# vincenthz/eccoxide

Measured on AMD Instinct MI355X. Metric: variable-base scalarmuls/sec (batch) per GPU + achieved HBM GB/s vs roofline, higher is better.
Workload: dtype u32

## Files before the change

### __graft_entry__.py

```python
import os
import subprocess
import sys

ROOT = os.path.dirname(os.path.abspath(__file__))
if ROOT not in sys.path:
    sys.path.insert(0, ROOT)


def build() -> None:
    jobs = str(min(6, os.cpu_count() or 1))
    subprocess.check_call(["make", "-C", os.path.join(ROOT, "eccoxide_amd", "csrc"), "-j", jobs, "ARCH=gfx950"])
    subprocess.check_call(["make", "-C", os.path.join(ROOT, "oracle")])
    subprocess.check_call(["make", "-C", os.path.join(ROOT, "tests", "cpp")])
    subprocess.check_call(["make", "-C", os.path.join(ROOT, "tests", "hip")])
    subprocess.check_call(["make", "-C", os.path.join(ROOT, "tests", "hip_p256k1")])
    subprocess.check_call(["make", "-C", os.path.join(ROOT, "tests", "hip_ed25519")])
    subprocess.check_call(["make", "-C", os.path.join(ROOT, "tests", "hip_merged")])
    subprocess.check_call(["make", "-C", os.path.join(ROOT, "tests", "hip_lo32")])
    subprocess.check_call(["make", "-C", os.path.join(ROOT, "tests", "hip_ecdsa")])
    subprocess.check_call(["make", "-C", os.path.join(ROOT, "tests", "hip_ed25519_sign")])
    subprocess.check_call(["make", "-C", os.path.join(ROOT, "tests", "hip_ecdsa_sign")])
    subprocess.check_call(["make", "-C", os.path.join(ROOT, "tests", "hip_h2c")])
    subprocess.check_call(["make", "-C", os.path.join(ROOT, "tests", "hip_g2")])
    subprocess.check_call(["make", "-C", os.path.join(ROOT, "tests", "hip_h2c_g2")])
    import eccoxide_amd
    from eccoxide_amd import _lib

    lib = _lib.load()
    assert lib.eccx_field_bytes(eccoxide_amd.P256R1) == 32


def smoke() -> None:
    import eccoxide_amd as E
    from eccoxide_amd import workload as W
    from tests import oracle_lib

    ora = oracle_lib.load()
    with E.Engine(0) as eng:
        for curve, n in (("p256r1", 300), ("ed25519", 300)):
            ks = W.random_scalars(curve, n, seed=1).tobytes()
            want_b = ora.base(curve, ks, threads=4)
            got_b = eng.scalarmul_base(curve, ks)
            assert got_b[0] == want_b[0] and got_b[1] == want_b[1], f"{curve}: fixed-base mismatch vs oracle"
            pts = want_b[0]
            ks2 = W.random_scalars(curve, n, seed=2).tobytes()
            want_v = ora.var(curve, ks2, pts, threads=4)
            got_d = eng.scalarmul_var(curve, ks2, pts)
            assert got_d[0] == want_v[0] and got_d[1] == want_v[1], f"{curve}: variable-base mismatch vs oracle"
            got_v = eng.scalarmul_var(curve, ks2, pts, want_proj=True)
            assert got_v[0] == want_v[0] and got_v[1] == want_v[1], f"{curve}: mirror variable-base mismatch vs oracle"
# ... 78 lines not shown
```

### eccoxide_amd/csrc/kernels_coz.hpp

```cpp
#pragma once
#include <type_traits>
#include "inv_gcd.hpp"
#include "kernels_ct.hpp"

namespace eccx {

struct NoGlv {
  static constexpr int K_BITS = 0;
};
struct PrimeOrderBases : NoGlv {};

template <class G>
ECCX_DEV void glv_split(uint32_t (&k1)[5], uint32_t (&k2)[5], const uint8_t* __restrict__ kb) {
  uint32_t k[8];
#pragma unroll
  for (int i = 0; i < 8; ++i) {
    const uint8_t* b = kb + 28 - 4 * i;
    k[i] = ((uint32_t)b[0] << 24) | ((uint32_t)b[1] << 16) | ((uint32_t)b[2] << 8) | (uint32_t)b[3];
  }
  uint32_t prod[13];
#pragma unroll
  for (int i = 0; i < 13; ++i) prod[i] = 0;
#pragma unroll
  for (int i = 0; i < 8; ++i) {
// ... 200 lines not shown
  constexpr uint32_t T = TAGGED ? CT_F32_TAG : 0u;
  uint32_t w[W];
#pragma unroll
  for (int i = 0; i < W; ++i) w[i] = (i < N ? x.v[i] : (i < 2 * N ? y.v[i - N] : 0u)) | T;
  uint4* dst = reinterpret_cast<uint4*>(row);
#pragma unroll
  for (int i = 0; i < W / 4; ++i) dst[i] = make_uint4(w[4 * i], w[4 * i + 1], w[4 * i + 2], w[4 * i + 3]);
}

template <class CU>
ECCX_DEV void ujac_madd_signed(UJac<CU>& r, bool& h_zero, bool& r_zero, const UJac<CU>& p,
                          const U<CU, 1, 3>& x2, const U<CU, 1, 3>& y2, bool neg) {
  auto z1z1 = u_sqr(p.z);
  auto u2 = u_mul(x2, z1z1);
  auto t = u_mul(p.z, z1z1);
  U<CU, 2, 4> sy;
  u_select(sy, neg, u_neg(y2), u_as<2, 4>(y2));
  auto s2 = u_mul(u_reduce(sy), t);
  auto h = u_reduce(u_sub(u2, p.x));
  auto rr = u_reduce(u_sub(s2, p.y));
  h_zero = u_is_zero_mod_p(h);
  r_zero = u_is_zero_mod_p(rr);
  auto hh = u_sqr(h);
  auto hhh = u_mul(h, hh);
  auto v = u_mul(p.x, hh);
  auto r2 = u_sqr(rr);
  auto x3 = u_reduce(u_sub(u_sub(u_sub(r2, hhh), v), v));
  r.x = x3;
  if constexpr (CU::KIND == UK_MONT) {
    r.y = u_fit<1, 3>(u_mul_add(rr, u_sub(v, x3), u_neg(p.y), hhh));
  } else if constexpr (UB<CU>::SPARSE) {
    r.y = u_mul_sub(rr, u_sub(v, x3), p.y, hhh);
  } else if constexpr (UBS<CU>::DENSE) {
    r.y = u_mul_sub(rr, u_reduce(u_sub(v, x3)), p.y, hhh);
  } else {
    auto y3a = u_mul(rr, u_sub(v, x3));
    auto y1h = u_mul(p.y, hhh);
    r.y = u_reduce(u_sub(y3a, y1h));
  }
  r.z = u_fit<UJac<CU>::ZK, UJac<CU>::ZV>(u_mul(p.z, h));
}

template <class CU>
ECCX_DEV void uzaddu(U<CU, 1, 3>& x1, U<CU, 1, 3>& y1, U<CU, 1, 3>& x2, U<CU, 1, 3>& y2, U<CU, 1, 3>& d_out, bool& d_zero) {
  const auto d = u_reduce(u_sub(x1, x2));
  d_zero = u_is_zero_mod_p(d);
  const auto c = u_sqr(d);
  const U<CU, 1, 3> w1 = u_fit<1, 3>(u_mul(x1, c));
  const auto w2 = u_mul(x2, c);
  const auto e = u_reduce(u_sub(y1, y2));
  const auto dd = u_sqr(e);
  const U<CU, 1, 3> a1 = u_fit<1, 3>(u_mul(y1, u_sub(w1, w2)));
  const auto x3 = u_reduce(u_sub(u_sub(dd, w1), w2));
  const auto y3m = u_mul(e, u_sub(w1, x3));
  x2 = x3;
  y2 = u_reduce(u_sub(y3m, a1));
  x1 = w1;
  y1 = a1;
  d_out = d;
}

template <class CU>
ECCX_DEV void ujac_madd_ct(UJac<CU>& r, bool& h_zero, bool& r_zero, const UJac<CU>& p, const U<CU, 1, 3>& x2,
                           const U<CU, 1, 3>& y2) {
  auto z1z1 = u_sqr(p.z);
  auto u2 = u_mul(x2, z1z1);
  auto t = u_mul(p.z, z1z1);
// ... 515 lines not shown
```

### eccoxide_amd/csrc/kernels_unsat.hpp

```cpp
#pragma once
#include "kernels_fast.hpp"
#include "ufe.hpp"

namespace eccx {
#ifndef ECCX_ENTRY_ALIGN
#define ECCX_ENTRY_ALIGN 32
#endif

template <class CU>
struct UJac {
  static constexpr int ZK = UB<CU>::KLAZY, ZV = ZK == 2 ? 4 : 3;
  U<CU, 1, 3> x, y;
  U<CU, ZK, ZV> z;
};

template <class CU>
struct UEntry {
  U<CU, 1, 3> x, y, z, zz, zzz;
};

template <class CU>
constexpr int urow3_words() { return ((3 * CU::N + 3) / 4) * 4; }
template <class CU>
ECCX_DEV void u3_store(uint32_t* __restrict__ row, const U<CU, 1, 3>& x, const U<CU, 1, 3>& y, const U<CU, 1, 3>& z) {
// ... 71 lines not shown
    r.x = x3;
    r.y = u_reduce(u_sub(u_sub(y3m, gg4), gg4));
    r.z = u_fit<UJac<CU>::ZK, UJac<CU>::ZV>(u_add(yz, yz));
  } else {
    auto delta = u_sqr(p.z);
    auto gamma = u_sqr(p.y);
    auto g2 = u_add(gamma, gamma);
    auto g4 = u_add(g2, g2);
    auto b4 = u_mul(p.x, g4);
    auto t1 = u_sub(p.x, delta);
    auto t2 = u_add(p.x, delta);
    auto t3 = u_mul(t1, t2);
    auto alpha = u_reduce(u_add(u_add(t3, t3), t3));
    auto x3a = u_sqr(alpha);
    auto x3 = u_reduce(u_sub(u_sub(x3a, b4), b4));
    auto yz = u_mul(p.y, p.z);
    auto t = u_sub(b4, x3);
    r.x = x3;
    if constexpr (UB<CU>::SPARSE) {
      r.y = u_mul_sub_2sqr(alpha, t, g2);
    } else {
      auto g8s = u_sqr(g2);
      auto y3m = u_mul(alpha, t);
      r.y = u_reduce(u_sub(u_sub(y3m, g8s), g8s));
    }
    r.z = u_fit<UJac<CU>::ZK, UJac<CU>::ZV>(u_add(yz, yz));
  }
}

template <class CU>
ECCX_DEV void ujac_dbl_merged(UJac<CU>& r, const UJac<CU>& p) {
  static_assert(UBS<CU>::DENSE && !CU::Sat::A0, "written for a = -3 on p = -1 mod 2^B without the sparse form");
  auto delta = u_sqr(p.z);
  auto gamma = u_sqr(p.y);
  auto g2 = u_reduce(u_add(gamma, gamma));
  auto g4 = u_add(g2, g2);
  auto b4 = u_mul(p.x, g4);
  auto t1 = u_sub(p.x, delta);
  auto t2 = u_add(p.x, delta);
  auto t3 = u_mul(t1, t2);
  auto alpha = u_reduce(u_add(u_add(t3, t3), t3));
  auto x3 = u_reduce(u_sub(u_sub(u_sqr(alpha), b4), b4));
  auto yz = u_mul(p.y, p.z);
  r.x = x3;
  r.y = u_mul_sub_2sqr(alpha, u_reduce(u_sub(b4, x3)), g2);
  r.z = u_fit<UJac<CU>::ZK, UJac<CU>::ZV>(u_add(yz, yz));
}

template <class CU>
ECCX_DEV void ujac_add_raw(UJac<CU>& r, bool& h_zero, bool& r_zero, U<CU, 1, 3>& ey, const UJac<CU>& p,
                           const UEntry<CU>& e, bool neg) {
  auto z1z1 = u_sqr(p.z);
  auto u1 = u_mul(p.x, e.zz);
  auto u2 = u_mul(e.x, z1z1);
  auto s1 = u_mul(p.y, e.zzz);
  auto t = u_mul(p.z, z1z1);
  U<CU, 2, 4> sy;
  u_select(sy, neg, u_neg(e.y), u_as<2, 4>(e.y));
  ey = u_reduce(sy);
  auto s2 = u_mul(ey, t);
  auto h = u_reduce(u_sub(u2, u1));
  auto rr = u_reduce(u_sub(s2, s1));
  h_zero = u_is_zero_mod_p(h);
  r_zero = u_is_zero_mod_p(rr);
  auto hh = u_sqr(h);
  auto hhh = u_mul(h, hh);
  auto v = u_mul(u1, hh);
  auto r2 = u_sqr(rr);
  auto x3 = u_reduce(u_sub(u_sub(u_sub(r2, hhh), v), v));
  auto tt = u_sub(v, x3);
  auto z3a = u_mul(p.z, e.z);
  r.x = x3;
  if constexpr (CU::KIND == UK_MONT) {
    r.y = u_fit<1, 3>(u_mul_add(rr, tt, u_neg(s1), hhh));
  } else if constexpr (UB<CU>::SPARSE) {
    r.y = u_mul_sub(rr, tt, s1, hhh);
  } else {
    auto y3a = u_mul(rr, tt);
// ... 1317 lines not shown
```

### eccoxide_amd/csrc/ufe.hpp

```cpp
#pragma once
#include "fe.hpp"

#include <type_traits>

#ifndef ECCX_SOLINAS_REDUCE
#define ECCX_SOLINAS_REDUCE 1
#endif

namespace eccx {

#include "umad_chunks.inc"

__device__ __forceinline__ void smad1_k(uint64_t& acc, uint32_t a, int32_t k) {
  asm("v_mad_i64_i32 %0, vcc, %1, %2, %0" : "+v"(acc) : "v"(a), "s"(k) : "vcc");
}

__device__ __forceinline__ void smad1_v(uint64_t& acc, int32_t a, int32_t b) {
  asm("v_mad_i64_i32 %0, vcc, %1, %2, %0" : "+v"(acc) : "v"(a), "v"(b) : "vcc");
}

template <int S>
__device__ __forceinline__ void ucarry_hi(uint64_t& acc) {
  uint64_t r;
  asm("v_mad_u64_u32 %0, vcc, %1, %2, 0" : "=&v"(r) : "v"((uint32_t)(acc >> 32)), "n"(1 << S) : "vcc");
// ... 123 lines not shown
  switch (q.n) {                                                                                                     \
    case 1: umad1_##SUF<F>(acc, h, ECCX_Q(0)); break;                                                              \
    case 2: umad2_##SUF<F>(acc, h, ECCX_Q(0), ECCX_Q(1)); break;                                                   \
    case 3: umad3_##SUF<F>(acc, h, ECCX_Q(0), ECCX_Q(1), ECCX_Q(2)); break;                                        \
    case 4: umad4_##SUF<F>(acc, h, ECCX_Q(0), ECCX_Q(1), ECCX_Q(2), ECCX_Q(3)); break;                             \
    case 5: umad5_##SUF<F>(acc, h, ECCX_Q(0), ECCX_Q(1), ECCX_Q(2), ECCX_Q(3), ECCX_Q(4)); break;                  \
    case 6: umad6_##SUF<F>(acc, h, ECCX_Q(0), ECCX_Q(1), ECCX_Q(2), ECCX_Q(3), ECCX_Q(4), ECCX_Q(5)); break;       \
    case 7: umad7_##SUF<F>(acc, h, ECCX_Q(0), ECCX_Q(1), ECCX_Q(2), ECCX_Q(3), ECCX_Q(4), ECCX_Q(5), ECCX_Q(6));   \
      break;                                                                                                       \
    case 8:                                                                                                        \
      umad8_##SUF<F>(acc, h, ECCX_Q(0), ECCX_Q(1), ECCX_Q(2), ECCX_Q(3), ECCX_Q(4), ECCX_Q(5), ECCX_Q(6), ECCX_Q(7)); \
      break;                                                                                                       \
    case 9:                                                                                                        \
      umad9_##SUF<F>(acc, h, ECCX_Q(0), ECCX_Q(1), ECCX_Q(2), ECCX_Q(3), ECCX_Q(4), ECCX_Q(5), ECCX_Q(6), ECCX_Q(7), \
                     ECCX_Q(8));                                                                                   \
      break;                                                                                                       \
    default:                                                                                                       \
      if (hc == 2) scarry_hi<S>(acc);                                                                              \
      else ucarry_hi<S>(acc);                                                                                      \
      break;                                                                                                       \
  }
    if constexpr (KC) {
      if (hc == 2) { ECCX_CHUNKS(ks) } else { ECCX_CHUNKS(kc) }
    } else {
      if (hc == 2) { ECCX_CHUNKS(vs) } else { ECCX_CHUNKS(vc) }
    }
#undef ECCX_CHUNKS
#undef ECCX_Q
    q.n = 0;
    hc = 0;
  }
};


template <class C, bool SQR, bool BCONST, bool LO32 = UB<C>::LO32>
ECCX_DEV void u_mul_core_mont(uint32_t (&r)[C::N], const uint32_t (&a)[C::N], const uint32_t (&b)[C::N]) {
  constexpr int N = C::N;
  constexpr bool PP1 = C::KIND == UK_MONT_PP1;
  auto PR = [](int j) constexpr { return PP1 ? C::PP1[j] : C::P[j]; };
  uint32_t m[N], t[N], a2[N];
  if constexpr (SQR) {
#pragma unroll
    for (int i = 0; i < N; ++i) a2[i] = a[i] << 1;
  }
  uint64_t acc = 0;
  std::conditional_t<UB<C>::LO32, UMacQC<BCONST, 32 - C::B>, UMacQ<BCONST>> qa;
  UMacQ<true> qm;
#pragma unroll
  for (int k = 0; k < 2 * N - 1; ++k) {
    const int lo = k < N ? 0 : k - N + 1, hi = k < N ? k : N - 1;
    if constexpr (SQR) {
#pragma unroll
      for (int i = lo; 2 * i < k; ++i) qa.push(acc, a[i], a2[k - i]);
      if ((k & 1) == 0) qa.push(acc, a[k / 2], a[k / 2]);
    } else {
#pragma unroll
      for (int i = lo; i <= hi; ++i) qa.push(acc, a[i], b[k - i]);
    }
    qa.flush(acc);
    if constexpr (UB<C>::SPARSE) {
#pragma unroll
      for (int t = 0; t < C::SPARSE_N; ++t) {
        const int i = k - C::SPARSE_OFF[t];
        if (i >= lo && i <= (k < N ? k - 1 : N - 1)) {
          if (C::SPARSE_SIGN[t] > 0) qm.push(acc, m[i], 1u << C::SPARSE_SHIFT[t]);
        }
      }
      qm.flush(acc);
#pragma unroll
      for (int t = 0; t < C::SPARSE_N; ++t) {
        const int i = k - C::SPARSE_OFF[t];
        if (i >= lo && i <= (k < N ? k - 1 : N - 1)) {
          if (C::SPARSE_SIGN[t] < 0) smad1_k(acc, m[i], -(int32_t)(1u << C::SPARSE_SHIFT[t]));
        }
      }
    } else {
#pragma unroll
      for (int i = lo; i <= (k < N ? k - 1 : N - 1); ++i) {
        if (PR(k - i) != 0) qm.push(acc, m[i], PR(k - i));
      }
      qm.flush(acc);
    }
    if constexpr (LO32) {
      if (k < N - 1) {
// ... 129 lines not shown
  for (int k = 0; k < 2 * N - 1; ++k) {
    const int lo = k < N ? 0 : k - N + 1, hi = k < N ? k : N - 1;
    if (k >= N) acc += (uint64_t)C::P[k - N];
#pragma unroll
    for (int i = lo; i <= hi; ++i) qa.push(acc, a[i], b[k - i]);
    qa.flush(acc);
    if constexpr (NEG_SQ) {
#pragma unroll
      for (int i = lo; 2 * i < k; ++i) smad1_v(acc, nc[i], (int32_t)(c[k - i] << 1));
      if ((k & 1) == 0) smad1_v(acc, nc[k / 2], (int32_t)c[k / 2]);
    } else {
#pragma unroll
      for (int i = lo; i <= hi; ++i) smad1_v(acc, nc[i], (int32_t)d[k - i]);
    }
#pragma unroll
    for (int i = lo; i <= (k < N ? k - 1 : N - 1); ++i) {
      if (C::P[k - i] != 0) qm.push(acc, m[i], C::P[k - i]);
    }
    qm.flush(acc);
    if (k < N) {
      m[k] = ((uint32_t)acc * C::N0B) & C::MASK;
      umad1_k(acc, m[k], C::P[0]);
    } else {
      t[k - N] = (uint32_t)acc & C::MASK;
    }
    acc = (uint64_t)((int64_t)acc >> C::B);
  }
  acc += (uint64_t)C::P[N - 1];
  t[N - 1] = (uint32_t)acc;
#pragma unroll
  for (int i = 0; i < N; ++i) r[i] = t[i];
}

template <class C, bool NEG_SQ>
ECCX_DEV void u_mul_sub_core_pp1(uint32_t (&r)[C::N], const uint32_t (&a)[C::N], const uint32_t (&b)[C::N],
                                 const uint32_t (&c)[C::N], const uint32_t (&d)[C::N]) {
  constexpr int N = C::N;
  static_assert(C::KIND == UK_MONT_PP1 && C::SPARSE_N == 0, "p = -1 mod 2^B with p + 1 as plain digits");
  uint32_t m[N], t[N];
  int32_t nc[N];
#pragma unroll
  for (int i = 0; i < N; ++i) nc[i] = NEG_SQ ? -(int32_t)(c[i] << 1) : -(int32_t)c[i];
  uint64_t acc = 0;
  UMacQC<false, 32 - C::B> qa;
  UMacQ<true> qm;
#pragma unroll
  for (int k = 0; k < 2 * N - 1; ++k) {
    const int lo = k < N ? 0 : k - N + 1, hi = k < N ? k : N - 1;
    if (k >= N && C::P[k - N] != 0) acc += (uint64_t)C::P[k - N];
#pragma unroll
    for (int i = lo; i <= hi; ++i) qa.push(acc, a[i], b[k - i]);
    qa.flush(acc);
    if constexpr (NEG_SQ) {
#pragma unroll
      for (int i = lo; 2 * i < k; ++i) smad1_v(acc, nc[i], (int32_t)(c[k - i] << 1));
      if ((k & 1) == 0) smad1_v(acc, nc[k / 2], (int32_t)c[k / 2]);
    } else {
#pragma unroll
      for (int i = lo; i <= hi; ++i) smad1_v(acc, nc[i], (int32_t)d[k - i]);
    }
#pragma unroll
    for (int i = lo; i <= (k < N ? k - 1 : N - 1); ++i) {
      if (C::PP1[k - i] != 0) qm.push(acc, m[i], C::PP1[k - i]);
    }
    qm.flush(acc);
    if (k < N - 1) {
      m[k] = (uint32_t)acc;
      qa.carry(acc, true);
      continue;
    }
    if (k < N) m[k] = (uint32_t)acc & C::MASK;
    else t[k - N] = (uint32_t)acc & C::MASK;
    acc = (uint64_t)((int64_t)acc >> C::B);
  }
  acc += (uint64_t)C::P[N - 1];
  t[N - 1] = (uint32_t)acc;
#pragma unroll
  for (int i = 0; i < N; ++i) r[i] = t[i];
}

template <class C, bool SQR, bool BCONST>
ECCX_DEV void u_mul_core_mers(uint32_t (&r)[C::N], const uint32_t (&a)[C::N], const uint32_t (&b)[C::N]) {
  constexpr int N = C::N;
  constexpr int S = C::B * N - C::PBITS;
  static_assert(S >= 1 && S <= 2, "wrap factor must keep shifted limbs below 2^32");
  uint32_t t[N], bw[N], a2[N];
#pragma unroll
  for (int i = 0; i < N; ++i) {
    if constexpr (SQR) {
      a2[i] = a[i] << 1;
      bw[i] = (S == 1) ? 0u : a[i] << (S + 1);
    } else {
      a2[i] = 0;
      bw[i] = b[i] << S;
    }
  }
  uint64_t acc = 0;
  UMacQ<BCONST && !SQR> qa;
  UMacQ<false> qw;
#pragma unroll
  for (int k = 0; k < N; ++k) {
// ... 197 lines not shown
  static constexpr bool DENSE = C::KIND == UK_MONT_PP1 && !UB<C>::SPARSE;
  static constexpr int KKS = (int)((~(uint64_t)0 >> 1) / ((uint64_t)C::N * UB<C>::COL)) - 1;
  static_assert(!DENSE || (uint64_t)C::N * KKS * UB<C>::COL <= (~(uint64_t)0 >> 1) - 0xffffffffull * UB<C>::pp1_sum() -
                                                                ((uint64_t)1 << C::B) - ((uint64_t)1 << (63 - C::B)),
                "32-bit Montgomery digits overflow the signed columns");
  static constexpr bool ks_ok(int k) { return ((uint64_t)(k + 1) << C::B) <= ((uint64_t)1 << 31); }
};

template <class C, int K1, int V1, int K2, int V2, int K3, int V3, int K4, int V4>
ECCX_DEV auto u_mul_sub(const U<C, K1, V1>& a, const U<C, K2, V2>& b, const U<C, K3, V3>& c, const U<C, K4, V4>& d) {
  static_assert(UBS<C>::OK || UBS<C>::DENSE, "implemented for the Montgomery fields with room for signed columns");
  static_assert(K1 * K2 <= UBS<C>::KKS && K3 * K4 <= UBS<C>::KKS, "a product overflows the signed columns");
  static_assert(UBS<C>::ks_ok(K3) && UBS<C>::ks_ok(K4), "negated / signed operands must stay below 2^31");
  static_assert((uint32_t)(V1 * V2) < C::RP && (uint32_t)(V3 * V4) < C::RP, "result outside (0, 3p)");
  U<C, 1, 3> r;
  if constexpr (UB<C>::SPARSE) u_mul_sub_core_sparse<C, false>(r.v, a.v, b.v, c.v, d.v);
  else if constexpr (UBS<C>::DENSE) u_mul_sub_core_pp1<C, false>(r.v, a.v, b.v, c.v, d.v);
  else u_mul_sub_core_mont<C, false>(r.v, a.v, b.v, c.v, d.v);
  return r;
}
template <class C, int K1, int V1, int K2, int V2, int K3, int V3>
ECCX_DEV auto u_mul_sub_2sqr(const U<C, K1, V1>& a, const U<C, K2, V2>& b, const U<C, K3, V3>& c) {
  static_assert(UBS<C>::OK || UBS<C>::DENSE, "implemented for the Montgomery fields with room for signed columns");
  static_assert(K1 * K2 <= UBS<C>::KKS && 2 * K3 * K3 <= UBS<C>::KKS, "a product overflows the signed columns");
  static_assert(UBS<C>::ks_ok(2 * K3), "doubled / negated operands must stay below 2^31");
  static_assert((uint32_t)(V1 * V2) < C::RP && (uint32_t)(2 * V3 * V3) < C::RP, "result outside (0, 3p)");
  U<C, 1, 3> r;
  if constexpr (UB<C>::SPARSE) u_mul_sub_core_sparse<C, true>(r.v, a.v, b.v, c.v, c.v);
  else if constexpr (UBS<C>::DENSE) u_mul_sub_core_pp1<C, true>(r.v, a.v, b.v, c.v, c.v);
  else u_mul_sub_core_mont<C, true>(r.v, a.v, b.v, c.v, c.v);
  return r;
}

template <class C, int K1, int V1>
ECCX_DEV auto u_sqr(const U<C, K1, V1>& a) {
  if constexpr (!UB<C>::ksq_ok(K1) || (UB<C>::vout(V1, V1) > 3)) {
    return u_sqr(u_reduce(a));
  } else {
    U<C, 1, UB<C>::vout(V1, V1)> r;
    u_mul_core<C, true, false>(r.v, a.v, a.v);
    return r;
  }
}

template <class C, int K1, int V1>
ECCX_DEV auto u_mul_k(const U<C, K1, V1>& a, const uint32_t (&k)[C::N]) {
  if constexpr (!UB<C>::kk_ok(K1, 1) || (UB<C>::vout(V1, 1) > 3)) {
    return u_mul_k(u_reduce(a), k);
  } else {
    U<C, 1, UB<C>::vout(V1, 1)> r;
    u_mul_core<C, false, true>(r.v, a.v, k);
    return r;
  }
}

template <class C>
ECCX_DEV U<C, 1, 2> u_mul_k_exit(const U<C, 1, 3>& a, const uint32_t (&k)[C::N]) {
  static_assert(UB<C>::MONT && UB<C>::vout(3, 1) <= 2, "Montgomery fields; a reduced operand times a constant below p");
  U<C, 1, 2> r;
  u_mul_core_mont<C, false, true, false>(r.v, a.v, k);
  return r;
}

template <class C, int K1, int V1>
ECCX_DEV U<C, 1, 2> u_mul_small(const U<C, K1, V1>& a, uint32_t k) {
  static_assert(C::KIND == UK_PM19, "written for 2^255 - 19");
// ... 217 lines not shown
```

### eccoxide_amd/csrc/umad_chunks.inc

```
__device__ __forceinline__ void umad1_v(uint64_t& acc, uint32_t a0, uint32_t b0) {
  asm("v_mad_u64_u32 %0, vcc, %1, %2, %0\n\t"
      : "+v"(acc)
      : "v"(a0), "v"(b0)
      : "vcc");
}
__device__ __forceinline__ void umad2_v(uint64_t& acc, uint32_t a0, uint32_t b0, uint32_t a1, uint32_t b1) {
  asm("v_mad_u64_u32 %0, vcc, %1, %2, %0\n\t"
      "v_mad_u64_u32 %0, vcc, %3, %4, %0\n\t"
      : "+v"(acc)
      : "v"(a0), "v"(b0), "v"(a1), "v"(b1)
      : "vcc");
}
__device__ __forceinline__ void umad3_v(uint64_t& acc, uint32_t a0, uint32_t b0, uint32_t a1, uint32_t b1, uint32_t a2, uint32_t b2) {
  asm("v_mad_u64_u32 %0, vcc, %1, %2, %0\n\t"
      "v_mad_u64_u32 %0, vcc, %3, %4, %0\n\t"
      "v_mad_u64_u32 %0, vcc, %5, %6, %0\n\t"
      : "+v"(acc)
      : "v"(a0), "v"(b0), "v"(a1), "v"(b1), "v"(a2), "v"(b2)
      : "vcc");
}
__device__ __forceinline__ void umad4_v(uint64_t& acc, uint32_t a0, uint32_t b0, uint32_t a1, uint32_t b1, uint32_t a2, uint32_t b2, uint32_t a3, uint32_t b3) {
  asm("v_mad_u64_u32 %0, vcc, %1, %2, %0\n\t"
      "v_mad_u64_u32 %0, vcc, %3, %4, %0\n\t"
      "v_mad_u64_u32 %0, vcc, %5, %6, %0\n\t"
// ... 554 lines not shown
      : "vcc");
}
template <int F>
__device__ __forceinline__ void umad8_ks(uint64_t& acc, uint32_t h, uint32_t a0, uint32_t b0, uint32_t a1, uint32_t b1, uint32_t a2, uint32_t b2, uint32_t a3, uint32_t b3, uint32_t a4, uint32_t b4, uint32_t a5, uint32_t b5, uint32_t a6, uint32_t b6, uint32_t a7, uint32_t b7) {
  asm("v_mad_i64_i32 %0, vcc, %1, %2, 0\n\t"
      "v_mad_u64_u32 %0, vcc, %3, %4, %0\n\t"
      "v_mad_u64_u32 %0, vcc, %5, %6, %0\n\t"
      "v_mad_u64_u32 %0, vcc, %7, %8, %0\n\t"
      "v_mad_u64_u32 %0, vcc, %9, %10, %0\n\t"
      "v_mad_u64_u32 %0, vcc, %11, %12, %0\n\t"
      "v_mad_u64_u32 %0, vcc, %13, %14, %0\n\t"
      "v_mad_u64_u32 %0, vcc, %15, %16, %0\n\t"
      "v_mad_u64_u32 %0, vcc, %17, %18, %0\n\t"
      : "=&v"(acc)
      : "v"(h), "n"(F), "v"(a0), "s"(b0), "v"(a1), "s"(b1), "v"(a2), "s"(b2), "v"(a3), "s"(b3), "v"(a4), "s"(b4), "v"(a5), "s"(b5), "v"(a6), "s"(b6), "v"(a7), "s"(b7)
      : "vcc");
}
template <int F>
__device__ __forceinline__ void umad9_ks(uint64_t& acc, uint32_t h, uint32_t a0, uint32_t b0, uint32_t a1, uint32_t b1, uint32_t a2, uint32_t b2, uint32_t a3, uint32_t b3, uint32_t a4, uint32_t b4, uint32_t a5, uint32_t b5, uint32_t a6, uint32_t b6, uint32_t a7, uint32_t b7, uint32_t a8, uint32_t b8) {
  asm("v_mad_i64_i32 %0, vcc, %1, %2, 0\n\t"
      "v_mad_u64_u32 %0, vcc, %3, %4, %0\n\t"
      "v_mad_u64_u32 %0, vcc, %5, %6, %0\n\t"
      "v_mad_u64_u32 %0, vcc, %7, %8, %0\n\t"
      "v_mad_u64_u32 %0, vcc, %9, %10, %0\n\t"
      "v_mad_u64_u32 %0, vcc, %11, %12, %0\n\t"
      "v_mad_u64_u32 %0, vcc, %13, %14, %0\n\t"
      "v_mad_u64_u32 %0, vcc, %15, %16, %0\n\t"
      "v_mad_u64_u32 %0, vcc, %17, %18, %0\n\t"
      "v_mad_u64_u32 %0, vcc, %19, %20, %0\n\t"
      : "=&v"(acc)
      : "v"(h), "n"(F), "v"(a0), "s"(b0), "v"(a1), "s"(b1), "v"(a2), "s"(b2), "v"(a3), "s"(b3), "v"(a4), "s"(b4), "v"(a5), "s"(b5), "v"(a6), "s"(b6), "v"(a7), "s"(b7), "v"(a8), "s"(b8)
      : "vcc");
}
```

Measured before the change: 77.11 million.

## Use signed limb differences in mul-sub and fused doubled square in Jacobian doubling

Adds a signed-limb type whose differences feed directly into the DENSE mul-sub kernel through signed 64-bit MADs. This drops the u_reduce after v-x3 and b4-x3 in the coZ add and merged doubling. Also adds u_sqr2, which computes 2*y^2 in one Montgomery square from pre-doubled operands instead of a square, an add and a reduce. In exchange the signed MAD chains need new overflow bounds, and these are checked with static_asserts.

```diff
diff --git a/__graft_entry__.py b/__graft_entry__.py
--- a/__graft_entry__.py
+++ b/__graft_entry__.py
@@ -16,6 +16,7 @@
     subprocess.check_call(["make", "-C", os.path.join(ROOT, "tests", "hip_p256k1")])
     subprocess.check_call(["make", "-C", os.path.join(ROOT, "tests", "hip_ed25519")])
     subprocess.check_call(["make", "-C", os.path.join(ROOT, "tests", "hip_merged")])
+    subprocess.check_call(["make", "-C", os.path.join(ROOT, "tests", "hip_signed")])
     subprocess.check_call(["make", "-C", os.path.join(ROOT, "tests", "hip_lo32")])
     subprocess.check_call(["make", "-C", os.path.join(ROOT, "tests", "hip_ecdsa")])
     subprocess.check_call(["make", "-C", os.path.join(ROOT, "tests", "hip_ed25519_sign")])
diff --git a/eccoxide_amd/csrc/kernels_coz.hpp b/eccoxide_amd/csrc/kernels_coz.hpp
--- a/eccoxide_amd/csrc/kernels_coz.hpp
+++ b/eccoxide_amd/csrc/kernels_coz.hpp
@@ -256,7 +256,7 @@
   } else if constexpr (UB<CU>::SPARSE) {
     r.y = u_mul_sub(rr, u_sub(v, x3), p.y, hhh);
   } else if constexpr (UBS<CU>::DENSE) {
-    r.y = u_mul_sub(rr, u_reduce(u_sub(v, x3)), p.y, hhh);
+    r.y = u_mul_sub(rr, u_sdiff(v, x3), p.y, hhh);
   } else {
     auto y3a = u_mul(rr, u_sub(v, x3));
     auto y1h = u_mul(p.y, hhh);
diff --git a/eccoxide_amd/csrc/kernels_unsat.hpp b/eccoxide_amd/csrc/kernels_unsat.hpp
--- a/eccoxide_amd/csrc/kernels_unsat.hpp
+++ b/eccoxide_amd/csrc/kernels_unsat.hpp
@@ -127,8 +127,7 @@
 ECCX_DEV void ujac_dbl_merged(UJac<CU>& r, const UJac<CU>& p) {
   static_assert(UBS<CU>::DENSE && !CU::Sat::A0, "written for a = -3 on p = -1 mod 2^B without the sparse form");
   auto delta = u_sqr(p.z);
-  auto gamma = u_sqr(p.y);
-  auto g2 = u_reduce(u_add(gamma, gamma));
+  auto g2 = u_sqr2(p.y);
   auto g4 = u_add(g2, g2);
   auto b4 = u_mul(p.x, g4);
   auto t1 = u_sub(p.x, delta);
@@ -138,7 +137,7 @@
   auto x3 = u_reduce(u_sub(u_sub(u_sqr(alpha), b4), b4));
   auto yz = u_mul(p.y, p.z);
   r.x = x3;
-  r.y = u_mul_sub_2sqr(alpha, u_reduce(u_sub(b4, x3)), g2);
+  r.y = u_mul_sub_2sqr(alpha, u_sdiff(b4, x3), g2);
   r.z = u_fit<UJac<CU>::ZK, UJac<CU>::ZV>(u_add(yz, yz));
 }
 
diff --git a/eccoxide_amd/csrc/ufe.hpp b/eccoxide_amd/csrc/ufe.hpp
--- a/eccoxide_amd/csrc/ufe.hpp
+++ b/eccoxide_amd/csrc/ufe.hpp
@@ -179,8 +179,59 @@
   }
 };
 
-
-template <class C, bool SQR, bool BCONST, bool LO32 = UB<C>::LO32>
+template <int S>
+struct UMacQS {
+  uint32_t x[9], y[9], h;
+  int n = 0;
+  bool hc = false;
+  ECCX_DEV void push(uint64_t& acc, uint32_t a, int32_t b) {
+    x[n] = a;
+    y[n] = (uint32_t)b;
+    if (++n == 9) flush(acc);
+  }
+  ECCX_DEV void carry(uint64_t acc) {
+    h = (uint32_t)(acc >> 32);
+    hc = true;
+  }
+  ECCX_DEV void flush(uint64_t& acc) {
+    static_assert(S >= 1 && S <= 6, "carry factor 2^S must be an inline constant");
+    constexpr int F = 1 << S;
+#define ECCX_Q(i) x[i], y[i]
+    if (hc) {
+      switch (n) {
+        case 1: umad1_vis<F>(acc, h, ECCX_Q(0)); break;
+        case 2: umad2_vis<F>(acc, h, ECCX_Q(0), ECCX_Q(1)); break;
+        case 3: umad3_vis<F>(acc, h, ECCX_Q(0), ECCX_Q(1), ECCX_Q(2)); break;
+        case 4: umad4_vis<F>(acc, h, ECCX_Q(0), ECCX_Q(1), ECCX_Q(2), ECCX_Q(3)); break;
+        case 5: umad5_vis<F>(acc, h, ECCX_Q(0), ECCX_Q(1), ECCX_Q(2), ECCX_Q(3), ECCX_Q(4)); break;
+        case 6: umad6_vis<F>(acc, h, ECCX_Q(0), ECCX_Q(1), ECCX_Q(2), ECCX_Q(3), ECCX_Q(4), ECCX_Q(5)); break;
+        case 7: umad7_vis<F>(acc, h, ECCX_Q(0), ECCX_Q(1), ECCX_Q(2), ECCX_Q(3), ECCX_Q(4), ECCX_Q(5), ECCX_Q(6)); break;
+        case 8: umad8_vis<F>(acc, h, ECCX_Q(0), ECCX_Q(1), ECCX_Q(2), ECCX_Q(3), ECCX_Q(4), ECCX_Q(5), ECCX_Q(6), ECCX_Q(7)); break;
+        case 9: umad9_vis<F>(acc, h, ECCX_Q(0), ECCX_Q(1), ECCX_Q(2), ECCX_Q(3), ECCX_Q(4), ECCX_Q(5), ECCX_Q(6), ECCX_Q(7), ECCX_Q(8)); break;
+        default: acc = (uint64_t)h << 32; scarry_hi<S>(acc); break;
+      }
+    } else {
+      switch (n) {
+        case 1: umad1_vi(acc, ECCX_Q(0)); break;
+        case 2: umad2_vi(acc, ECCX_Q(0), ECCX_Q(1)); break;
+        case 3: umad3_vi(acc, ECCX_Q(0), ECCX_Q(1), ECCX_Q(2)); break;
+        case 4: umad4_vi(acc, ECCX_Q(0), ECCX_Q(1), ECCX_Q(2), ECCX_Q(3)); break;
+        case 5: umad5_vi(acc, ECCX_Q(0), ECCX_Q(1), ECCX_Q(2), ECCX_Q(3), ECCX_Q(4)); break;
+        case 6: umad6_vi(acc, ECCX_Q(0), ECCX_Q(1), ECCX_Q(2), ECCX_Q(3), ECCX_Q(4), ECCX_Q(5)); break;
+        case 7: umad7_vi(acc, ECCX_Q(0), ECCX_Q(1), ECCX_Q(2), ECCX_Q(3), ECCX_Q(4), ECCX_Q(5), ECCX_Q(6)); break;
+        case 8: umad8_vi(acc, ECCX_Q(0), ECCX_Q(1), ECCX_Q(2), ECCX_Q(3), ECCX_Q(4), ECCX_Q(5), ECCX_Q(6), ECCX_Q(7)); break;
+        case 9: umad9_vi(acc, ECCX_Q(0), ECCX_Q(1), ECCX_Q(2), ECCX_Q(3), ECCX_Q(4), ECCX_Q(5), ECCX_Q(6), ECCX_Q(7), ECCX_Q(8)); break;
+        default: break;
+      }
+    }
+#undef ECCX_Q
+    n = 0;
+    hc = false;
+  }
+};
+
+
+template <class C, bool SQR, bool BCONST, bool LO32 = UB<C>::LO32, bool DBL = false>
 ECCX_DEV void u_mul_core_mont(uint32_t (&r)[C::N], const uint32_t (&a)[C::N], const uint32_t (&b)[C::N]) {
   constexpr int N = C::N;
   constexpr bool PP1 = C::KIND == UK_MONT_PP1;
@@ -196,7 +247,11 @@
 #pragma unroll
   for (int k = 0; k < 2 * N - 1; ++k) {
     const int lo = k < N ? 0 : k - N + 1, hi = k < N ? k : N - 1;
-    if constexpr (SQR) {
+    if constexpr (SQR && DBL) {
+#pragma unroll
+      for (int i = lo; 2 * i < k; ++i) qa.push(acc, a2[i], a2[k - i]);
+      if ((k & 1) == 0) qa.push(acc, a[k / 2], a2[k / 2]);
+    } else if constexpr (SQR) {
 #pragma unroll
       for (int i = lo; 2 * i < k; ++i) qa.push(acc, a[i], a2[k - i]);
       if ((k & 1) == 0) qa.push(acc, a[k / 2], a[k / 2]);
@@ -392,17 +447,19 @@
   for (int i = 0; i < N; ++i) r[i] = t[i];
 }
 
-template <class C, bool NEG_SQ>
-ECCX_DEV void u_mul_sub_core_pp1(uint32_t (&r)[C::N], const uint32_t (&a)[C::N], const uint32_t (&b)[C::N],
+template <class C, bool NEG_SQ, class TB = uint32_t>
+ECCX_DEV void u_mul_sub_core_pp1(uint32_t (&r)[C::N], const uint32_t (&a)[C::N], const TB (&b)[C::N],
                                  const uint32_t (&c)[C::N], const uint32_t (&d)[C::N]) {
   constexpr int N = C::N;
+  constexpr bool BS = std::is_same_v<TB, int32_t>;
+  static_assert(BS || std::is_same_v<TB, uint32_t>, "second factor: unsigned limbs or signed differences");
   static_assert(C::KIND == UK_MONT_PP1 && C::SPARSE_N == 0, "p = -1 mod 2^B with p + 1 as plain digits");
   uint32_t m[N], t[N];
   int32_t nc[N];
 #pragma unroll
   for (int i = 0; i < N; ++i) nc[i] = NEG_SQ ? -(int32_t)(c[i] << 1) : -(int32_t)c[i];
   uint64_t acc = 0;
-  UMacQC<false, 32 - C::B> qa;
+  std::conditional_t<BS, UMacQS<32 - C::B>, UMacQC<false, 32 - C::B>> qa;
   UMacQ<true> qm;
 #pragma unroll
   for (int k = 0; k < 2 * N - 1; ++k) {
@@ -426,7 +483,8 @@
     qm.flush(acc);
     if (k < N - 1) {
       m[k] = (uint32_t)acc;
-      qa.carry(acc, true);
+      if constexpr (BS) qa.carry(acc);
+      else qa.carry(acc, true);
       continue;
     }
     if (k < N) m[k] = (uint32_t)acc & C::MASK;
@@ -690,6 +748,60 @@
   return r;
 }
 
+template <class C, int K, int V>
+struct US {
+  static_assert(K >= 1 && UBS<C>::ks_ok(K), "signed limbs must stay below 2^31");
+  static_assert(V >= 1 && V <= 4096, "value bound out of range");
+  int32_t v[C::N];
+};
+
+template <class C, int V1, int V2>
+ECCX_DEV auto u_sdiff(const U<C, 1, V1>& a, const U<C, 1, V2>& b) {
+  US<C, 1, (V1 > V2 ? V1 : V2)> r;
+#pragma unroll
+  for (int i = 0; i < C::N; ++i) r.v[i] = (int32_t)(a.v[i] - b.v[i]);
+  return r;
+}
+
+template <class C>
+constexpr bool ubs_neg_side_ok(int kk) {
+  return (uint64_t)C::N * (uint64_t)kk * UB<C>::COL <= (~(uint64_t)0 >> 1) - ((uint64_t)1 << (64 - C::B));
+}
+
+template <class C, int K1, int V1, int K2, int V2, int K3, int V3, int K4, int V4>
+ECCX_DEV auto u_mul_sub(const U<C, K1, V1>& a, const US<C, K2, V2>& b, const U<C, K3, V3>& c, const U<C, K4, V4>& d) {
+  static_assert(UBS<C>::DENSE, "signed operands are implemented for p = -1 mod 2^B with p + 1 as plain digits");
+  static_assert(K1 * K2 <= UBS<C>::KKS && K3 * K4 <= UBS<C>::KKS, "a product overflows the signed columns");
+  static_assert(UBS<C>::ks_ok(K1) && UBS<C>::ks_ok(K3) && UBS<C>::ks_ok(K4), "negated / signed operands must stay below 2^31");
+  static_assert(ubs_neg_side_ok<C>(K1 * K2 + K3 * K4), "the negative side of a column overflows");
+  static_assert((uint32_t)(V1 * V2 + V3 * V4) < C::RP, "result outside (0, 3p)");
+  U<C, 1, 3> r;
+  u_mul_sub_core_pp1<C, false, int32_t>(r.v, a.v, b.v, c.v, d.v);
+  return r;
+}
+template <class C, int K1, int V1, int K2, int V2, int K3, int V3>
+ECCX_DEV auto u_mul_sub_2sqr(const U<C, K1, V1>& a, const US<C, K2, V2>& b, const U<C, K3, V3>& c) {
+  static_assert(UBS<C>::DENSE, "signed operands are implemented for p = -1 mod 2^B with p + 1 as plain digits");
+  static_assert(K1 * K2 <= UBS<C>::KKS && 2 * K3 * K3 <= UBS<C>::KKS, "a product overflows the signed columns");
+  static_assert(UBS<C>::ks_ok(K1) && UBS<C>::ks_ok(2 * K3), "doubled / negated operands must stay below 2^31");
+  static_assert(ubs_neg_side_ok<C>(K1 * K2 + 2 * K3 * K3), "the negative side of a column overflows");
+  static_assert((uint32_t)(V1 * V2 + 2 * V3 * V3) < C::RP, "result outside (0, 3p)");
+  U<C, 1, 3> r;
+  u_mul_sub_core_pp1<C, true, int32_t>(r.v, a.v, b.v, c.v, c.v);
+  return r;
+}
+
+template <class C, int V1>
+ECCX_DEV auto u_sqr2(const U<C, 1, V1>& a) {
+  static_assert(UBS<C>::DENSE && UB<C>::LO32, "written for p = -1 mod 2^B with p + 1 as plain digits");
+  static_assert(UB<C>::kk_ok(2, 1), "columns: a square with doubled terms carries a product with K1*K2 = 2");
+  static_assert(UB<C>::KMAX >= 2, "limbs: the doubled operand a << 1 (below 2 * 2^B) stays below 2^32");
+  static_assert(UB<C>::vout(2 * V1, V1) <= 3, "result too large: reduce the operand first");
+  U<C, 1, UB<C>::vout(2 * V1, V1)> r;
+  u_mul_core_mont<C, true, false, true, true>(r.v, a.v, a.v);
+  return r;
+}
+
 template <class C, int K1, int V1>
 ECCX_DEV auto u_sqr(const U<C, K1, V1>& a) {
   if constexpr (!UB<C>::ksq_ok(K1) || (UB<C>::vout(V1, V1) > 3)) {
diff --git a/eccoxide_amd/csrc/umad_chunks.inc b/eccoxide_amd/csrc/umad_chunks.inc
--- a/eccoxide_amd/csrc/umad_chunks.inc
+++ b/eccoxide_amd/csrc/umad_chunks.inc
@@ -610,3 +610,201 @@
       : "v"(h), "n"(F), "v"(a0), "s"(b0), "v"(a1), "s"(b1), "v"(a2), "s"(b2), "v"(a3), "s"(b3), "v"(a4), "s"(b4), "v"(a5), "s"(b5), "v"(a6), "s"(b6), "v"(a7), "s"(b7), "v"(a8), "s"(b8)
       : "vcc");
 }
+__device__ __forceinline__ void umad1_vi(uint64_t& acc, uint32_t a0, uint32_t b0) {
+  asm("v_mad_i64_i32 %0, vcc, %1, %2, %0\n\t"
+      : "+v"(acc)
+      : "v"(a0), "v"(b0)
+      : "vcc");
+}
+__device__ __forceinline__ void umad2_vi(uint64_t& acc, uint32_t a0, uint32_t b0, uint32_t a1, uint32_t b1) {
+  asm("v_mad_i64_i32 %0, vcc, %1, %2, %0\n\t"
+      "v_mad_i64_i32 %0, vcc, %3, %4, %0\n\t"
+      : "+v"(acc)
+      : "v"(a0), "v"(b0), "v"(a1), "v"(b1)
+      : "vcc");
+}
+__device__ __forceinline__ void umad3_vi(uint64_t& acc, uint32_t a0, uint32_t b0, uint32_t a1, uint32_t b1, uint32_t a2, uint32_t b2) {
+  asm("v_mad_i64_i32 %0, vcc, %1, %2, %0\n\t"
+      "v_mad_i64_i32 %0, vcc, %3, %4, %0\n\t"
+      "v_mad_i64_i32 %0, vcc, %5, %6, %0\n\t"
+      : "+v"(acc)
+      : "v"(a0), "v"(b0), "v"(a1), "v"(b1), "v"(a2), "v"(b2)
+      : "vcc");
+}
+__device__ __forceinline__ void umad4_vi(uint64_t& acc, uint32_t a0, uint32_t b0, uint32_t a1, uint32_t b1, uint32_t a2, uint32_t b2, uint32_t a3, uint32_t b3) {
+  asm("v_mad_i64_i32 %0, vcc, %1, %2, %0\n\t"
+      "v_mad_i64_i32 %0, vcc, %3, %4, %0\n\t"
+      "v_mad_i64_i32 %0, vcc, %5, %6, %0\n\t"
+      "v_mad_i64_i32 %0, vcc, %7, %8, %0\n\t"
+      : "+v"(acc)
+      : "v"(a0), "v"(b0), "v"(a1), "v"(b1), "v"(a2), "v"(b2), "v"(a3), "v"(b3)
+      : "vcc");
+}
+__device__ __forceinline__ void umad5_vi(uint64_t& acc, uint32_t a0, uint32_t b0, uint32_t a1, uint32_t b1, uint32_t a2, uint32_t b2, uint32_t a3, uint32_t b3, uint32_t a4, uint32_t b4) {
+  asm("v_mad_i64_i32 %0, vcc, %1, %2, %0\n\t"
+      "v_mad_i64_i32 %0, vcc, %3, %4, %0\n\t"
+      "v_mad_i64_i32 %0, vcc, %5, %6, %0\n\t"
+      "v_mad_i64_i32 %0, vcc, %7, %8, %0\n\t"
+      "v_mad_i64_i32 %0, vcc, %9, %10, %0\n\t"
+      : "+v"(acc)
+      : "v"(a0), "v"(b0), "v"(a1), "v"(b1), "v"(a2), "v"(b2), "v"(a3), "v"(b3), "v"(a4), "v"(b4)
+      : "vcc");
+}
+__device__ __forceinline__ void umad6_vi(uint64_t& acc, uint32_t a0, uint32_t b0, uint32_t a1, uint32_t b1, uint32_t a2, uint32_t b2, uint32_t a3, uint32_t b3, uint32_t a4, uint32_t b4, uint32_t a5, uint32_t b5) {
+  asm("v_mad_i64_i32 %0, vcc, %1, %2, %0\n\t"
+      "v_mad_i64_i32 %0, vcc, %3, %4, %0\n\t"
+      "v_mad_i64_i32 %0, vcc, %5, %6, %0\n\t"
+      "v_mad_i64_i32 %0, vcc, %7, %8, %0\n\t"
+      "v_mad_i64_i32 %0, vcc, %9, %10, %0\n\t"
+      "v_mad_i64_i32 %0, vcc, %11, %12, %0\n\t"
+      : "+v"(acc)
+      : "v"(a0), "v"(b0), "v"(a1), "v"(b1), "v"(a2), "v"(b2), "v"(a3), "v"(b3), "v"(a4), "v"(b4), "v"(a5), "v"(b5)
+      : "vcc");
+}
+__device__ __forceinline__ void umad7_vi(uint64_t& acc, uint32_t a0, uint32_t b0, uint32_t a1, uint32_t b1, uint32_t a2, uint32_t b2, uint32_t a3, uint32_t b3, uint32_t a4, uint32_t b4, uint32_t a5, uint32_t b5, uint32_t a6, uint32_t b6) {
+  asm("v_mad_i64_i32 %0, vcc, %1, %2, %0\n\t"
+      "v_mad_i64_i32 %0, vcc, %3, %4, %0\n\t"
+      "v_mad_i64_i32 %0, vcc, %5, %6, %0\n\t"
+      "v_mad_i64_i32 %0, vcc, %7, %8, %0\n\t"
+      "v_mad_i64_i32 %0, vcc, %9, %10, %0\n\t"
+      "v_mad_i64_i32 %0, vcc, %11, %12, %0\n\t"
+      "v_mad_i64_i32 %0, vcc, %13, %14, %0\n\t"
+      : "+v"(acc)
+      : "v"(a0), "v"(b0), "v"(a1), "v"(b1), "v"(a2), "v"(b2), "v"(a3), "v"(b3), "v"(a4), "v"(b4), "v"(a5), "v"(b5), "v"(a6), "v"(b6)
+      : "vcc");
+}
+__device__ __forceinline__ void umad8_vi(uint64_t& acc, uint32_t a0, uint32_t b0, uint32_t a1, uint32_t b1, uint32_t a2, uint32_t b2, uint32_t a3, uint32_t b3, uint32_t a4, uint32_t b4, uint32_t a5, uint32_t b5, uint32_t a6, uint32_t b6, uint32_t a7, uint32_t b7) {
+  asm("v_mad_i64_i32 %0, vcc, %1, %2, %0\n\t"
+      "v_mad_i64_i32 %0, vcc, %3, %4, %0\n\t"
+      "v_mad_i64_i32 %0, vcc, %5, %6, %0\n\t"
+      "v_mad_i64_i32 %0, vcc, %7, %8, %0\n\t"
+      "v_mad_i64_i32 %0, vcc, %9, %10, %0\n\t"
+      "v_mad_i64_i32 %0, vcc, %11, %12, %0\n\t"
+      "v_mad_i64_i32 %0, vcc, %13, %14, %0\n\t"
+      "v_mad_i64_i32 %0, vcc, %15, %16, %0\n\t"
+      : "+v"(acc)
+      : "v"(a0), "v"(b0), "v"(a1), "v"(b1), "v"(a2), "v"(b2), "v"(a3), "v"(b3), "v"(a4), "v"(b4), "v"(a5), "v"(b5), "v"(a6), "v"(b6), "v"(a7), "v"(b7)
+      : "vcc");
+}
+__device__ __forceinline__ void umad9_vi(uint64_t& acc, uint32_t a0, uint32_t b0, uint32_t a1, uint32_t b1, uint32_t a2, uint32_t b2, uint32_t a3, uint32_t b3, uint32_t a4, uint32_t b4, uint32_t a5, uint32_t b5, uint32_t a6, uint32_t b6, uint32_t a7, uint32_t b7, uint32_t a8, uint32_t b8) {
+  asm("v_mad_i64_i32 %0, vcc, %1, %2, %0\n\t"
+      "v_mad_i64_i32 %0, vcc, %3, %4, %0\n\t"
+      "v_mad_i64_i32 %0, vcc, %5, %6, %0\n\t"
+      "v_mad_i64_i32 %0, vcc, %7, %8, %0\n\t"
+      "v_mad_i64_i32 %0, vcc, %9, %10, %0\n\t"
+      "v_mad_i64_i32 %0, vcc, %11, %12, %0\n\t"
+      "v_mad_i64_i32 %0, vcc, %13, %14, %0\n\t"
+      "v_mad_i64_i32 %0, vcc, %15, %16, %0\n\t"
+      "v_mad_i64_i32 %0, vcc, %17, %18, %0\n\t"
+      : "+v"(acc)
+      : "v"(a0), "v"(b0), "v"(a1), "v"(b1), "v"(a2), "v"(b2), "v"(a3), "v"(b3), "v"(a4), "v"(b4), "v"(a5), "v"(b5), "v"(a6), "v"(b6), "v"(a7), "v"(b7), "v"(a8), "v"(b8)
+      : "vcc");
+}
+template <int F>
+__device__ __forceinline__ void umad1_vis(uint64_t& acc, uint32_t h, uint32_t a0, uint32_t b0) {
+  asm("v_mad_i64_i32 %0, vcc, %1, %2, 0\n\t"
+      "v_mad_i64_i32 %0, vcc, %3, %4, %0\n\t"
+      : "=&v"(acc)
+      : "v"(h), "n"(F), "v"(a0), "v"(b0)
+      : "vcc");
+}
+template <int F>
+__device__ __forceinline__ void umad2_vis(uint64_t& acc, uint32_t h, uint32_t a0, uint32_t b0, uint32_t a1, uint32_t b1) {
+  asm("v_mad_i64_i32 %0, vcc, %1, %2, 0\n\t"
+      "v_mad_i64_i32 %0, vcc, %3, %4, %0\n\t"
+      "v_mad_i64_i32 %0, vcc, %5, %6, %0\n\t"
+      : "=&v"(acc)
+      : "v"(h), "n"(F), "v"(a0), "v"(b0), "v"(a1), "v"(b1)
+      : "vcc");
+}
+template <int F>
+__device__ __forceinline__ void umad3_vis(uint64_t& acc, uint32_t h, uint32_t a0, uint32_t b0, uint32_t a1, uint32_t b1, uint32_t a2, uint32_t b2) {
+  asm("v_mad_i64_i32 %0, vcc, %1, %2, 0\n\t"
+      "v_mad_i64_i32 %0, vcc, %3, %4, %0\n\t"
+      "v_mad_i64_i32 %0, vcc, %5, %6, %0\n\t"
+      "v_mad_i64_i32 %0, vcc, %7, %8, %0\n\t"
+      : "=&v"(acc)
+      : "v"(h), "n"(F), "v"(a0), "v"(b0), "v"(a1), "v"(b1), "v"(a2), "v"(b2)
+      : "vcc");
+}
+template <int F>
+__device__ __forceinline__ void umad4_vis(uint64_t& acc, uint32_t h, uint32_t a0, uint32_t b0, uint32_t a1, uint32_t b1, uint32_t a2, uint32_t b2, uint32_t a3, uint32_t b3) {
+  asm("v_mad_i64_i32 %0, vcc, %1, %2, 0\n\t"
+      "v_mad_i64_i32 %0, vcc, %3, %4, %0\n\t"
+      "v_mad_i64_i32 %0, vcc, %5, %6, %0\n\t"
+      "v_mad_i64_i32 %0, vcc, %7, %8, %0\n\t"
+      "v_mad_i64_i32 %0, vcc, %9, %10, %0\n\t"
+      : "=&v"(acc)
+      : "v"(h), "n"(F), "v"(a0), "v"(b0), "v"(a1), "v"(b1), "v"(a2), "v"(b2), "v"(a3), "v"(b3)
+      : "vcc");
+}
+template <int F>
+__device__ __forceinline__ void umad5_vis(uint64_t& acc, uint32_t h, uint32_t a0, uint32_t b0, uint32_t a1, uint32_t b1, uint32_t a2, uint32_t b2, uint32_t a3, uint32_t b3, uint32_t a4, uint32_t b4) {
+  asm("v_mad_i64_i32 %0, vcc, %1, %2, 0\n\t"
+      "v_mad_i64_i32 %0, vcc, %3, %4, %0\n\t"
+      "v_mad_i64_i32 %0, vcc, %5, %6, %0\n\t"
+      "v_mad_i64_i32 %0, vcc, %7, %8, %0\n\t"
+      "v_mad_i64_i32 %0, vcc, %9, %10, %0\n\t"
+      "v_mad_i64_i32 %0, vcc, %11, %12, %0\n\t"
+      : "=&v"(acc)
+      : "v"(h), "n"(F), "v"(a0), "v"(b0), "v"(a1), "v"(b1), "v"(a2), "v"(b2), "v"(a3), "v"(b3), "v"(a4), "v"(b4)
+      : "vcc");
+}
+template <int F>
+__device__ __forceinline__ void umad6_vis(uint64_t& acc, uint32_t h, uint32_t a0, uint32_t b0, uint32_t a1, uint32_t b1, uint32_t a2, uint32_t b2, uint32_t a3, uint32_t b3, uint32_t a4, uint32_t b4, uint32_t a5, uint32_t b5) {
+  asm("v_mad_i64_i32 %0, vcc, %1, %2, 0\n\t"
+      "v_mad_i64_i32 %0, vcc, %3, %4, %0\n\t"
+      "v_mad_i64_i32 %0, vcc, %5, %6, %0\n\t"
+      "v_mad_i64_i32 %0, vcc, %7, %8, %0\n\t"
+      "v_mad_i64_i32 %0, vcc, %9, %10, %0\n\t"
+      "v_mad_i64_i32 %0, vcc, %11, %12, %0\n\t"
+      "v_mad_i64_i32 %0, vcc, %13, %14, %0\n\t"
+      : "=&v"(acc)
+      : "v"(h), "n"(F), "v"(a0), "v"(b0), "v"(a1), "v"(b1), "v"(a2), "v"(b2), "v"(a3), "v"(b3), "v"(a4), "v"(b4), "v"(a5), "v"(b5)
+      : "vcc");
+}
+template <int F>
+__device__ __forceinline__ void umad7_vis(uint64_t& acc, uint32_t h, uint32_t a0, uint32_t b0, uint32_t a1, uint32_t b1, uint32_t a2, uint32_t b2, uint32_t a3, uint32_t b3, uint32_t a4, uint32_t b4, uint32_t a5, uint32_t b5, uint32_t a6, uint32_t b6) {
+  asm("v_mad_i64_i32 %0, vcc, %1, %2, 0\n\t"
+      "v_mad_i64_i32 %0, vcc, %3, %4, %0\n\t"
+      "v_mad_i64_i32 %0, vcc, %5, %6, %0\n\t"
+      "v_mad_i64_i32 %0, vcc, %7, %8, %0\n\t"
+      "v_mad_i64_i32 %0, vcc, %9, %10, %0\n\t"
+      "v_mad_i64_i32 %0, vcc, %11, %12, %0\n\t"
+      "v_mad_i64_i32 %0, vcc, %13, %14, %0\n\t"
+      "v_mad_i64_i32 %0, vcc, %15, %16, %0\n\t"
+      : "=&v"(acc)
+      : "v"(h), "n"(F), "v"(a0), "v"(b0), "v"(a1), "v"(b1), "v"(a2), "v"(b2), "v"(a3), "v"(b3), "v"(a4), "v"(b4), "v"(a5), "v"(b5), "v"(a6), "v"(b6)
+      : "vcc");
+}
+template <int F>
+__device__ __forceinline__ void umad8_vis(uint64_t& acc, uint32_t h, uint32_t a0, uint32_t b0, uint32_t a1, uint32_t b1, uint32_t a2, uint32_t b2, uint32_t a3, uint32_t b3, uint32_t a4, uint32_t b4, uint32_t a5, uint32_t b5, uint32_t a6, uint32_t b6, uint32_t a7, uint32_t b7) {
+  asm("v_mad_i64_i32 %0, vcc, %1, %2, 0\n\t"
+      "v_mad_i64_i32 %0, vcc, %3, %4, %0\n\t"
+      "v_mad_i64_i32 %0, vcc, %5, %6, %0\n\t"
+      "v_mad_i64_i32 %0, vcc, %7, %8, %0\n\t"
+      "v_mad_i64_i32 %0, vcc, %9, %10, %0\n\t"
+      "v_mad_i64_i32 %0, vcc, %11, %12, %0\n\t"
+      "v_mad_i64_i32 %0, vcc, %13, %14, %0\n\t"
+      "v_mad_i64_i32 %0, vcc, %15, %16, %0\n\t"
+      "v_mad_i64_i32 %0, vcc, %17, %18, %0\n\t"
+      : "=&v"(acc)
+      : "v"(h), "n"(F), "v"(a0), "v"(b0), "v"(a1), "v"(b1), "v"(a2), "v"(b2), "v"(a3), "v"(b3), "v"(a4), "v"(b4), "v"(a5), "v"(b5), "v"(a6), "v"(b6), "v"(a7), "v"(b7)
+      : "vcc");
+}
+template <int F>
+__device__ __forceinline__ void umad9_vis(uint64_t& acc, uint32_t h, uint32_t a0, uint32_t b0, uint32_t a1, uint32_t b1, uint32_t a2, uint32_t b2, uint32_t a3, uint32_t b3, uint32_t a4, uint32_t b4, uint32_t a5, uint32_t b5, uint32_t a6, uint32_t b6, uint32_t a7, uint32_t b7, uint32_t a8, uint32_t b8) {
+  asm("v_mad_i64_i32 %0, vcc, %1, %2, 0\n\t"
+      "v_mad_i64_i32 %0, vcc, %3, %4, %0\n\t"
+      "v_mad_i64_i32 %0, vcc, %5, %6, %0\n\t"
+      "v_mad_i64_i32 %0, vcc, %7, %8, %0\n\t"
+      "v_mad_i64_i32 %0, vcc, %9, %10, %0\n\t"
+      "v_mad_i64_i32 %0, vcc, %11, %12, %0\n\t"
+      "v_mad_i64_i32 %0, vcc, %13, %14, %0\n\t"
+      "v_mad_i64_i32 %0, vcc, %15, %16, %0\n\t"
+      "v_mad_i64_i32 %0, vcc, %17, %18, %0\n\t"
+      "v_mad_i64_i32 %0, vcc, %19, %20, %0\n\t"
+      : "=&v"(acc)
+      : "v"(h), "n"(F), "v"(a0), "v"(b0), "v"(a1), "v"(b1), "v"(a2), "v"(b2), "v"(a3), "v"(b3), "v"(a4), "v"(b4), "v"(a5), "v"(b5), "v"(a6), "v"(b6), "v"(a7), "v"(b7), "v"(a8), "v"(b8)
+      : "vcc");
+}
```

Measured after the change: 78.61 million, median of 6. 1.02x the previous value.
